# Nightmare-n/GD-MAE

Hardware: AMD Instinct MI355X
Metric: MAE pre-train frames/sec (Waymo-shape, 180k pts, 75% mask) (higher is better)
Workload: dtype bf16

## Files before the change

### gd-mae_amd/csrc/conv_tiles.hip

```cpp
#include "conv_tiles.h"

typedef float f32x16 __attribute__((ext_vector_type(16)));
typedef __bf16 bf16x8 __attribute__((ext_vector_type(8)));
typedef _Float16 f16x8 __attribute__((ext_vector_type(8)));
union CtFrag {
  uint4 q;
  bf16x8 v;
  f16x8 h;
};

#define CT_C 128
#define CT_SITE_PITCH 272
#ifndef CT_CH
#define CT_CH 128
#endif
#ifndef CT_RING
#define CT_RING 8
#endif
#define CT_HALVES (CT_C / CT_CH)
#define CT_KS (CT_CH / 16)
#define CT_NSTEP (9 * CT_KS)
#define CT_CPS (CT_CH / 8)
#define CT_PSITE (CT_CH * 2 + 16)
#define CT_ROW_PITCH (CT_CH == 128 ? 2944 : 1664)
// ... 540 lines not shown
#undef CT_STAGE
  }
  __syncthreads();
  float* red = (float*)(lds + CT_RED_OFF);
  const int elc = tid & 15, elsg = tid >> 4;
#pragma unroll
  for (int t = 0; t < CT_TPW; ++t) {
    if (!have[t]) continue;
    float s[8], q2[8];
#pragma unroll
    for (int j = 0; j < 8; ++j) s[j] = q2[j] = 0.f;
#pragma unroll
    for (int p = 0; p < 64 / CT_ESPP; ++p) {
      const int site = p * CT_ESPP + elsg;
      const uint4 v = *(const uint4*)(lds + t * CT_STAGE_PITCH + site * CT_SITE_PITCH + elc * 16);
      *(uint4*)(A.Yc + ((long long)slot[t] * GD_TILE_SITES + site) * CT_C + elc * 8) = v;
      if (ty0[t] + (site >> 3) < A.H && tx0[t] + (site & 7) < A.W) {
        float f[8];
        ct_unpack8(v, f);
#pragma unroll
        for (int j = 0; j < 8; ++j) {
          s[j] += f[j];
          q2[j] = fmaf(f[j], f[j], q2[j]);
        }
      }
    }
#pragma unroll
    for (int j = 0; j < 8; ++j) {
      s[j] += __shfl_xor(s[j], 16, 64);
      s[j] += __shfl_xor(s[j], 32, 64);
      q2[j] += __shfl_xor(q2[j], 16, 64);
      q2[j] += __shfl_xor(q2[j], 32, 64);
    }
    if (lane < 16) {
#pragma unroll
      for (int j = 0; j < 8; ++j) {
        red[((t * CT_NWAVES + wvg) * 2 + 0) * CT_C + elc * 8 + j] = s[j];
        red[((t * CT_NWAVES + wvg) * 2 + 1) * CT_C + elc * 8 + j] = q2[j];
      }
    }
  }
  __syncthreads();
#pragma unroll
  for (int t = 0; t < CT_TPW; ++t) {
    if (!have[t] || tid >= 256) continue;
    const int stat = tid >> 7, ch = tid & 127;
    float v = 0.f;
#pragma unroll
    for (int w = 0; w < CT_NWAVES; ++w) v += red[((t * CT_NWAVES + w) * 2 + stat) * CT_C + ch];
    A.part[(long long)slot[t] * 256 + tid] = v;
  }
}

__global__ __launch_bounds__(256) void k_ct_stats_reduce(const float* __restrict__ part, int n_act, const int* __restrict__ tile_list,
                                                         const unsigned short* __restrict__ ybg, int B, int H, int W, int TH, int TW,
                                                         float* __restrict__ red) {
  const int tid = threadIdx.x;
  if ((int)blockIdx.x < CT_NRED) {
    const int chunk = (n_act + CT_NRED - 1) / CT_NRED;
    const int r0 = blockIdx.x * chunk, r1 = r0 + chunk < n_act ? r0 + chunk : n_act;
    float a0 = 0.f, a1 = 0.f, a2 = 0.f, a3 = 0.f;
    int r = r0;
    for (; r + 15 < r1; r += 16) {
      float v[16];
#pragma unroll
      for (int u = 0; u < 16; ++u) v[u] = part[(long long)(r + u) * 256 + tid];
#pragma unroll
      for (int u = 0; u < 16; u += 4) {
        a0 += v[u];
        a1 += v[u + 1];
        a2 += v[u + 2];
        a3 += v[u + 3];
      }
    }
    for (; r + 3 < r1; r += 4) {
      a0 += part[(long long)r * 256 + tid];
      a1 += part[(long long)(r + 1) * 256 + tid];
      a2 += part[(long long)(r + 2) * 256 + tid];
      a3 += part[(long long)(r + 3) * 256 + tid];
    }
    for (; r < r1; ++r) a0 += part[(long long)r * 256 + tid];
    red[(long long)blockIdx.x * 256 + tid] = (a0 + a1) + (a2 + a3);
    return;
  }
  __shared__ int cnt[9];
  if (tid < 9) cnt[tid] = 0;
  __syncthreads();
  int c[9];
#pragma unroll
  for (int k = 0; k < 9; ++k) c[k] = 0;
  for (int i0 = tid; i0 < n_act; i0 += 8 * 256) {
   int tl[8];
#pragma unroll
   for (int u = 0; u < 8; ++u) tl[u] = tile_list[i0 + u * 256 < n_act ? i0 + u * 256 : n_act - 1];
#pragma unroll
   for (int u = 0; u < 8; ++u) {
    if (i0 + u * 256 >= n_act) continue;
    const int tile = tl[u];
    const int tx = tile % TW, ty = (tile / TW) % TH;
    const int y0 = ty * 8, y1 = y0 + 8 < H ? y0 + 8 : H, x0 = tx * 8, x1 = x0 + 8 < W ? x0 + 8 : W;
    const int ry[3] = {y0 == 0 ? 1 : 0, 0, y1 == H ? 1 : 0};
    const int rx[3] = {x0 == 0 ? 1 : 0, 0, x1 == W ? 1 : 0};
    const int my = (y1 - y0) - ry[0] - ry[2], mx = (x1 - x0) - rx[0] - rx[2];
#pragma unroll
    for (int cy = 0; cy < 3; ++cy)
#pragma unroll
      for (int cx = 0; cx < 3; ++cx) c[cy * 3 + cx] += (cy == 1 ? my : ry[cy]) * (cx == 1 ? mx : rx[cx]);
   }
  }
#pragma unroll
  for (int k = 0; k < 9; ++k)
    if (c[k]) atomicAdd(&cnt[k], c[k]);
  __syncthreads();
  const int stat = tid >> 7, ch = tid & 127;
  double acc = 0.0;
#pragma unroll
  for (int cy = 0; cy < 3; ++cy)
#pragma unroll
    for (int cx = 0; cx < 3; ++cx) {
      const long long total = (long long)B * (cy == 1 ? H - 2 : 1) * (cx == 1 ? W - 2 : 1);
      const double n = (double)(total - cnt[cy * 3 + cx]);
      const double v = (double)ct_bf2f(ybg[(cy * 3 + cx) * CT_C + ch]);
      acc += n * (stat ? v * v : v);
    }
  const float hi = (float)acc;
  red[(long long)CT_NRED * 256 + tid] = hi;
  red[(long long)(CT_NRED + 1) * 256 + tid] = (float)(acc - (double)hi);
}

int gd_bn_fold_from_partials(hipStream_t st, const float* part, int nblk, int C, double count, const float* gamma,
                             const float* beta, double eps, double momentum, float* running_mean, float* running_var,
                             long long* num_batches, double* stats, float* ab, float* mv);

extern "C" size_t gdmae_conv3x3_tiles_workspace_bytes(int n_act) {
  return gd_align((size_t)(n_act > 0 ? n_act : 1) * 256 * sizeof(float)) + gd_align((size_t)(CT_NRED + 2) * 256 * sizeof(float));
}

static int ct_fwd(const void* const* P, const int* const* maps, const float* const* a, const float* const* b, const int* strides, int k,
                  const void* Wp, const void* ybg, const int* tile_list, int n_act, int B, int H, int W, void* Yc, const float* gamma,
                  const float* beta, double eps, double momentum, float* running_mean, float* running_var, long long* num_batches,
                  double* stats, float* ab, float* mv, const int* tile_class, const int* tile_order, const float* pre, void* workspace,
                  void* stream) {
  GD_REQUIRE(k >= 1 && k <= CT_MAX_SRC, "conv3x3_tiles: 1..3 source stages");
  GD_REQUIRE(H >= 2 && W >= 2, "conv3x3_tiles: map too small");
  hipStream_t st = (hipStream_t)stream;
  CtArgs A;
  A.k = k;
  for (int g = 0; g < CT_MAX_SRC; ++g) {
    if (g < k) {
      const int s = strides[g];
      GD_REQUIRE((s == 1 || s == 2 || s == 4 || s == 8) && H % s == 0 && W % s == 0, "conv3x3_tiles: stride");
      A.src[g].P = (const unsigned short*)P[g];
      A.src[g].map = maps[g];
      A.src[g].a = a[g];
      A.src[g].b = b[g];
      A.src[g].ls = s == 1 ? 0 : (s == 2 ? 1 : (s == 4 ? 2 : 3));
    } else {
      A.src[g].P = nullptr; A.src[g].map = nullptr; A.src[g].a = nullptr; A.src[g].b = nullptr; A.src[g].ls = 0;
    }
  }
  A.Wp = (const uint4*)Wp;
  A.tile_list = tile_list;
  A.n_act = n_act;
  A.H = H; A.W = W; A.TH = (H + 7) / 8; A.TW = (W + 7) / 8;
  A.Yc = (unsigned short*)Yc;
  A.tile_class = CT_SKIP_OK ? tile_class : nullptr;
  A.tile_order = CT_SKIP_OK ? tile_order : nullptr;
  A.pre = CT_SKIP_OK ? pre : nullptr;
  GdArena ar(workspace, gdmae_conv3x3_tiles_workspace_bytes(n_act));
  float* part = ar.take<float>((size_t)(n_act > 0 ? n_act : 1) * 256);
  float* red = ar.take<float>((size_t)(CT_NRED + 2) * 256);
  A.part = part;
  if (n_act > 0) {
    static bool once = false;
    if (!once) {
      GD_CHECK(hipFuncSetAttribute((const void*)k_conv3x3_tiles, hipFuncAttributeMaxDynamicSharedMemorySize, CT_LDS_BYTES));
      once = true;
    }
    hipLaunchKernelGGL(k_conv3x3_tiles, dim3((n_act + CT_TPW - 1) / CT_TPW), dim3(CT_THREADS), CT_LDS_BYTES, st, A);
    GD_LAUNCH_CHECK();
  }
  hipLaunchKernelGGL(k_ct_stats_reduce, dim3(CT_NRED + 1), dim3(256), 0, st, (const float*)part, n_act, tile_list,
                     (const unsigned short*)ybg, B, H, W, A.TH, A.TW, red);
  GD_LAUNCH_CHECK();
  return gd_bn_fold_from_partials(st, red, CT_NRED + 2, CT_C, (double)B * H * W, gamma, beta, eps, momentum, running_mean,
                                  running_var, num_batches, stats, ab, mv);
}

extern "C" int gdmae_conv3x3_tiles_fwd(const void* const* P, const int* const* maps, const float* const* a, const float* const* b,
                                       const int* strides, int k, const void* Wp, const void* ybg, const int* tile_list, int n_act,
                                       int B, int H, int W, void* Yc, const float* gamma, const float* beta, double eps,
                                       double momentum, float* running_mean, float* running_var, long long* num_batches,
                                       double* stats, float* ab, float* mv, void* workspace, void* stream) {
  return ct_fwd(P, maps, a, b, strides, k, Wp, ybg, tile_list, n_act, B, H, W, Yc, gamma, beta, eps, momentum, running_mean, running_var,
                num_batches, stats, ab, mv, nullptr, nullptr, nullptr, workspace, stream);
}

extern "C" int gdmae_conv3x3_tiles_fwd_skip(const void* const* P, const int* const* maps, const float* const* a, const float* const* b,
                                            const int* strides, int k, const void* Wp, const void* ybg, const int* tile_list, int n_act,
                                            int B, int H, int W, void* Yc, const float* gamma, const float* beta, double eps,
                                            double momentum, float* running_mean, float* running_var, long long* num_batches,
                                            double* stats, float* ab, float* mv, const int* tile_class, const int* tile_order,
                                            const float* pre, void* workspace, void* stream) {
  const bool none = !tile_class && !tile_order && !pre;
  GD_REQUIRE(none || (tile_class && tile_order && (pre || k < 2)), "conv3x3_tiles_fwd_skip: tile_class, tile_order and pre, or none of them");
  return ct_fwd(P, maps, a, b, strides, k, Wp, ybg, tile_list, n_act, B, H, W, Yc, gamma, beta, eps, momentum, running_mean, running_var,
                num_batches, stats, ab, mv, tile_class, tile_order, pre, workspace, stream);
}

template <int ES>
__global__ __launch_bounds__(256) void k_tiles_gather_rows(const void* __restrict__ Yc, GdTiles T, const int* __restrict__ cell,
                                                           long long n, int H, int W, int C, uint4* __restrict__ out) {
  const int cv = C * ES / 16;
  const long long total = n * cv;
  for (long long i = blockIdx.x * (long long)blockDim.x + threadIdx.x; i < total; i += (long long)gridDim.x * blockDim.x) {
    const long long r = total < (1ll << 31) ? (long long)((unsigned)i / (unsigned)cv) : i / cv;
    const int v = (int)(i - r * cv);
    const int s = cell[r];
    const int x = s % W, q = s / W, y = q % H, b = q / H;
    out[i] = ((const uint4*)gd_y_row<ES>(Yc, T, b, y, x, H, W, C))[v];
  }
}

extern "C" int gdmae_tiles_gather_rows(const void* Yc, const int* tile_slot, const void* ybg, const int* cell, long long n, int H,
                                       int W, int C, int elem_bytes, void* out, void* stream) {
  GD_REQUIRE(tile_slot != nullptr && (elem_bytes == 2 || elem_bytes == 4) && (C * elem_bytes) % 16 == 0, "tiles_gather_rows");
  if (n <= 0) return 0;
  GdTiles T{tile_slot, ybg, (H + 7) / 8, (W + 7) / 8};
  long long g = (n * (C * elem_bytes / 16) + 255) / 256;
  if (g > 16384) g = 16384;
  if (elem_bytes == 2) hipLaunchKernelGGL(k_tiles_gather_rows<2>, dim3((int)g), dim3(256), 0, (hipStream_t)stream, Yc, T, cell, n, H, W, C, (uint4*)out);
  else hipLaunchKernelGGL(k_tiles_gather_rows<4>, dim3((int)g), dim3(256), 0, (hipStream_t)stream, Yc, T, cell, n, H, W, C, (uint4*)out);
  GD_LAUNCH_CHECK();
  return 0;
}

__global__ __launch_bounds__(256) void k_tiles_gather_rows_affine_relu(const void* __restrict__ Yc, GdTiles T, const int* __restrict__ cell,
                                                                       long long n, int H, int W, int C, const float* __restrict__ a,
                                                                       const float* __restrict__ b, uint4* __restrict__ yrows,
                                                                       float4* __restrict__ out) {
  const int cv = C / 8;
  const long long total = n * cv;
  for (long long i = blockIdx.x * (long long)blockDim.x + threadIdx.x; i < total; i += (long long)gridDim.x * blockDim.x) {
    const long long r = total < (1ll << 31) ? (long long)((unsigned)i / (unsigned)cv) : i / cv;
    const int v = (int)(i - r * cv);
    const int s = cell[r];
    const int x = s % W, q = s / W, y = q % H, bb = q / H;
    const uint4 yq = ((const uint4*)gd_y_row<2>(Yc, T, bb, y, x, H, W, C))[v];
    const float4 a0 = ((const float4*)a)[2 * v], a1 = ((const float4*)a)[2 * v + 1];
    const float4 b0 = ((const float4*)b)[2 * v], b1 = ((const float4*)b)[2 * v + 1];
    const unsigned w4[4] = {yq.x, yq.y, yq.z, yq.w};
    const float av[8] = {a0.x, a0.y, a0.z, a0.w, a1.x, a1.y, a1.z, a1.w};
    const float bv[8] = {b0.x, b0.y, b0.z, b0.w, b1.x, b1.y, b1.z, b1.w};
    float o[8];
#pragma unroll
    for (int j = 0; j < 4; ++j) {
      const float h0 = fmaf(av[2 * j], __uint_as_float(w4[j] << 16), bv[2 * j]);
      const float h1 = fmaf(av[2 * j + 1], __uint_as_float(w4[j] & 0xFFFF0000u), bv[2 * j + 1]);
      o[2 * j] = h0 > 0.f ? h0 : 0.f;
      o[2 * j + 1] = h1 > 0.f ? h1 : 0.f;
// ... 86 lines not shown
```

### gd-mae_amd/gdmae_hip/lib.py

```python
from __future__ import annotations

import ctypes as C
import os

import torch

_HERE = os.path.dirname(os.path.abspath(__file__))
LIB_PATH = os.path.abspath(os.path.join(_HERE, "..", "csrc", "libgdmae_hip.so"))
if os.environ.get("GDMAE_LIB"):
    LIB_PATH = os.path.abspath(os.environ["GDMAE_LIB"])


class GdmaeHipError(RuntimeError):
    pass


_P, _I, _L, _F, _D, _Z = C.c_void_p, C.c_int, C.c_longlong, C.c_float, C.c_double, C.c_size_t

SIGNATURES = {
    "gdmae_abi_version": (_I, []),
    "gdmae_target_arch": (C.c_char_p, []),
    "gdmae_last_error": (C.c_char_p, []),
    "gdmae_voxelize_workspace_bytes": (_Z, [_L, _I, _I, _I, _I]),
    "gdmae_voxelize": (_I, [_P, _L, _I, _P, _P, _P, _I, _P, _P, _P, _P, _P, _P, _P, _P, _P, _P, _P, _P, _P, _P, _Z, _P]),
# ... 4 lines not shown
    "gdmae_vfe_point_layer_fwd": (_I, [_P, _P, _P, _P, _I, _L, _I, _P, _P, _P, _I, _P, _P, _D, _D, _P, _P, _P, _P, _P, _P, _P, _I, _P, _P]),
    "gdmae_vfe_point_layer_bwd": (_I, [_P, _P, _P, _P, _I, _L, _I, _P, _P, _P, _I, _P, _P, _P, _P, _I, _P, _P, _P, _I, _P, _P]),
    "gdmae_vfe_max_layer_workspace_bytes": (_Z, []),
    "gdmae_vfe_max_layer_fwd": (_I, [_P, _L, _P, _P, _P, _I, _P, _P, _D, _D, _P, _P, _P, _P, _P, _P, _P, _P, _P, _P]),
    "gdmae_vfe_max_layer_bwd": (_I, [_P, _L, _P, _P, _I, _P, _P, _P, _P, _P, _P, _P, _P, _P, _P, _P, _I, _P, _P]),
    "gdmae_vfe_max_layer_fwd_f16": (_I, [_P, _L, _P, _P, _P, _I, _P, _P, _D, _D, _P, _P, _P, _P, _P, _P, _P, _P, _P, _P]),
    "gdmae_vfe_max_layer_bwd_f16": (_I, [_P, _L, _P, _P, _I, _P, _P, _P, _P, _P, _P, _P, _P, _P, _P, _P, _I, _P, _P]),
    "gdmae_vfe_max_layer_vis_fwd": (_I, [_P, _L, _P, _P, _P, _L, _I, _P, _P, _D, _D, _P, _P, _P, _P, _P, _P, _P, _P, _P, _P]),
    "gdmae_vfe_max_layer_vis_fwd_f16": (_I, [_P, _L, _P, _P, _P, _L, _I, _P, _P, _D, _D, _P, _P, _P, _P, _P, _P, _P, _P, _P, _P]),
    "gdmae_vfe_max_layer_vis_bwd": (_I, [_P, _L, _P, _P, _P, _I, _I, _P, _P, _P, _P, _P, _P, _P, _P, _P, _P, _P, _I, _P, _P]),
    "gdmae_vfe_max_layer_vis_bwd_f16": (_I, [_P, _L, _P, _P, _P, _I, _I, _P, _P, _P, _P, _P, _P, _P, _P, _P, _P, _P, _I, _P, _P]),
    "gdmae_fill_rows": (_I, [_P, _L, _I, _I, _P, _P]),
    "gdmae_weighted_mean_finish": (_I, [_P, _P, _L, _P, _P]),
    "gdmae_decoder_region_workspace_bytes": (_Z, [_I, _I]),
    "gdmae_decoder_region_algebra": (_I, [_P, _P, _P, _P, _P, _P, _P, _D, _I, _I, _P, _P, _I, _P, _P, _P, _P, _P, _P]),
    "gdmae_segment_max": (_I, [_P, _P, _P, _I, _I, _P, _P, _P]),
    "gdmae_segment_max_bwd": (_I, [_P, _P, _P, _L, _I, _P, _P]),
    "gdmae_random_mask": (_I, [_P, _P, _I, _D, _P, _P, _P]),
    "gdmae_visible_tokens": (_I, [_P, _P, _P, _L, _L, _P, _P, _P, _P, _P, _P]),
    "gdmae_downsample_tokens": (_I, [_P, _P, _L, _I, _I, _I, _P, _P, _P, _P, _P, _P]),
    "gdmae_rulebook": (_I, [_P, _P, _L, _I, _I, _I, _I, _I, _P, _I, _P, _P]),
    "gdmae_window_workspace_bytes": (_Z, [_I, _I, _I, _I, _I]),
    "gdmae_window_partition": (_I, [_P, _I, _I, _I, _I, _I, _I, _I, _P, _P, _P, _P, _P, _P, _P, _P, _P, _P, _P, _P, _Z, _P]),
    "gdmae_gather_rows": (_I, [_P, _P, _L, _I, _P, _P]),
    "gdmae_scatter_rows": (_I, [_P, _P, _L, _I, _P, _P]),
    "gdmae_gather_rows_strided": (_I, [_P, _P, _L, _I, _I, _I, _P, _P]),
    "gdmae_scatter_rows_strided": (_I, [_P, _P, _L, _I, _I, _I, _P, _P]),
    "gdmae_colstats_workspace_bytes": (_Z, [_I]),
    "gdmae_colstats": (_I, [_P, _L, _I, _I, _P, _P, _P]),
    "gdmae_rows_affine_relu_scatter": (_I, [_P, _I, _P, _L, _I, _P, _P, _P, _I, _I, _I, _P]),
    "gdmae_rows_affine_relu_sub": (_I, [_P, _I, _P, _L, _I, _P, _P, _P, _P, _I, _I, _I, _P]),
    "gdmae_rows_affine_relu_add": (_I, [_P, _I, _L, _I, _P, _P, _P, _P, _I, _P]),
    "gdmae_rows_bwd_stats_workspace_bytes": (_Z, [_I]),
    "gdmae_rows_bwd_stats": (_I, [_P, _I, _P, _L, _I, _P, _P, _P, _I, _I, _I, _P, _P, _P]),
    "gdmae_bn_fold": (_I, [_P, _L, _I, _I, _D, _P, _P, _D, _D, _P, _P, _P, _P, _P, _P, _P, _P]),
    "gdmae_bn_bwd_coeffs": (_I, [_P, _I, _P, _P, _P, _I, _D, _P, _P, _P, _I, _P, _P]),
    "gdmae_rows_bwd_stats_rows": (_I, [_L]),
    "gdmae_bn_bwd_coeffs_rows": (_I, [_P, _I, _I, _P, _P, _P, _I, _D, _P, _P, _P, _I, _P, _P]),
    "gdmae_border_sums_workspace_bytes": (_Z, [_I, _I]),
    "gdmae_border_sums": (_I, [_P, _I, _P, _P, _P, _P, _I, _I, _I, _I, _I, _P, _P, _P]),
    "gdmae_border_sums_rows": (_I, [_P, _I, _P, _P, _P, _P, _P, _P, _P, _I, _I, _I, _I, _I, _P, _P, _P]),
    "gdmae_conv3x3_grad_taps": (_I, [_P, _I, _P, _P, _P, _P, _P, _P, _P, _L, _I, _I, _I, _P, _P]),
    "gdmae_decoder_tiles_workspace_bytes": (_Z, [_I, _I, _I]),
    "gdmae_decoder_tiles": (_I, [_P, _P, _I, _I, _I, _I, _P, _P, _P, _P, _P]),
    "gdmae_conv3x3_tiles_packed_bytes": (_Z, [_I]),
    "gdmae_conv3x3_tiles_pack": (_I, [_P, _I, _I, _P, _I, _P, _P, _P, _P]),
    "gdmae_conv3x3_tiles_workspace_bytes": (_Z, [_I]),
    "gdmae_conv3x3_tiles_fwd": (_I, [_P, _P, _P, _P, _P, _I, _P, _P, _P, _I, _I, _I, _I, _P, _P, _P, _D, _D, _P, _P, _P, _P, _P, _P,
                                     _P, _P]),
    "gdmae_decoder_tiles_classes": (_I, [_P, _P, _I, _I, _I, _I, _P, _P, _P, _P, _P, _P, _P]),
    "gdmae_conv3x3_tiles_pack_pre": (_I, [_P, _I, _I, _P, _I, _P, _P, _P, _P, _P]),
    "gdmae_conv3x3_tiles_fwd_skip": (_I, [_P, _P, _P, _P, _P, _I, _P, _P, _P, _I, _I, _I, _I, _P, _P, _P, _D, _D, _P, _P, _P, _P, _P, _P,
                                          _P, _P, _P, _P, _P]),
    "gdmae_tiles_gather_rows": (_I, [_P, _P, _P, _P, _L, _I, _I, _I, _I, _P, _P]),
    "gdmae_tiles_gather_rows_affine_relu": (_I, [_P, _P, _P, _P, _L, _I, _I, _I, _P, _P, _P, _P, _P]),
    "gdmae_tiles_to_dense": (_I, [_P, _P, _P, _I, _I, _I, _I, _I, _P, _P]),
    "gdmae_tiles_to_dense_affine_relu": (_I, [_P, _P, _P, _I, _I, _I, _I, _P, _P, _P, _P]),
    "gdmae_rows_bwd": (_I, [_P, _I, _P, _L, _I, _P, _P, _P, _P, _P, _I, _I, _I, _P, _I, _P]),
    "gdmae_segment_max_affine": (_I, [_P, _I, _P, _P, _I, _I, _P, _P, _P, _P, _P]),
    "gdmae_segmax_bwd_stats": (_I, [_P, _I, _P, _P, _P, _L, _I, _P, _P, _P, _P, _P]),
    "gdmae_segmax_bn_bwd": (_I, [_P, _I, _P, _P, _P, _P, _L, _I, _P, _P, _P, _P, _I, _P]),
    "gdmae_window_attention_fwd": (_I, [_P, _P, _P, _I, _P, _P, _P, _I, _I, _I, _I, _P, _F, _P]),
    "gdmae_window_attention_bwd": (_I, [_P, _P, _P, _P, _P, _I, _P, _P, _P, _P, _I, _I, _I, _I, _P, _F, _P]),
    "gdmae_window_attention_levels_writes_lse": (_I, [_I, _I, _P, _I, _I]),
    "gdmae_window_attention_levels_fwd": (_I, [_P, _P, _P, _I, _P, _P, _P, _I, _P, _P, _I, _I, _P, _F, _P, _P]),
    "gdmae_window_attention_levels_bwd": (_I, [_P, _P, _P, _P, _P, _I, _P, _P, _P, _P, _I, _P, _P, _I, _I, _P, _F, _P, _P, _P]),
    "gdmae_conv3x3_dense_packed_bytes": (_Z, [_I, _I]),
    "gdmae_conv3x3_dense_pack": (_I, [_P, _I, _I, _I, _I, _P, _P]),
    "gdmae_conv3x3_dense": (_I, [_P, _I, _I, _I, _I, _I, _I, _P, _P, _P, _P]),
    "gdmae_conv3x3_dense_add": (_I, [_P, _I, _I, _I, _I, _I, _I, _P, _P, _P, _P, _P]),
    "gdmae_conv3x3_dense_relu": (_I, [_P, _I, _I, _I, _I, _I, _I, _P, _P, _P, _P, _P]),
    "gdmae_conv3x3_dense_stats_workspace_bytes": (_Z, [_I, _I, _I, _I]),
    "gdmae_conv3x3_dense_stat_rows": (_I, []),
    "gdmae_conv3x3_dense_stats": (_I, [_P, _I, _I, _I, _I, _I, _I, _P, _P, _P, _P, _P, _P]),
    "gdmae_bn_fold_partials": (_I, [_P, _I, _I, _D, _P, _P, _D, _D, _P, _P, _P, _P, _P, _P, _P]),
    "gdmae_conv3x3_dense_f32out": (_I, [_P, _I, _I, _I, _I, _I, _I, _P, _P, _P, _I, _P]),
    "gdmae_conv3x3_dense_dw_workspace_bytes": (_Z, [_I, _I, _I, _I, _I]),
    "gdmae_conv3x3_dense_bwd_weight": (_I, [_P, _P, _I, _I, _I, _I, _I, _I, _I, _I, _P, _P, _P]),
    "gdmae_attention_timing": (_I, [_I]),
    "gdmae_attention_timing_read": (_I, [_I, _P, _P]),
    "gdmae_kernel_timing": (_I, [_I]),
    "gdmae_kernel_timing_slots": (_I, []),
    "gdmae_kernel_timing_name": (C.c_char_p, [_I]),
    "gdmae_kernel_timing_read": (_I, [_I, _P, _P, _P, _P]),
    "gdmae_kernel_timing_read_side": (_I, [_I, _P]),
    "gdmae_add_layernorm_workspace_bytes": (_Z, [_I]),
    "gdmae_add_layernorm_fwd": (_I, [_P, _P, _I, _P, _P, _L, _I, _F, _P, _P, _P, _P]),
    "gdmae_add_layernorm_bwd": (_I, [_P, _P, _I, _P, _P, _P, _P, _I, _L, _I, _P, _P, _P, _P, _P]),
    "gdmae_prep_tokens": (_I, [_P, _P, _P, _L, _I, _P, _P, _I, _P]),
    "gdmae_sum_bf16": (_I, [_P, _I, _L, _P, _P]),
    "gdmae_add3": (_I, [_P, _P, _I, _P, _I, _L, _P, _P]),
    "gdmae_add3_to": (_I, [_P, _P, _I, _P, _I, _L, _P, _I, _P]),
    "gdmae_set_attention_impl": (_I, [_I]),
    "gdmae_sum_partials": (_I, [_P, _L, _F, _P, _I, _P]),
    "gdmae_sum_partials_gated": (_I, [_P, _L, _F, _P, _P, _F, _P]),
    "gdmae_gemm_workspace_bytes": (_Z, []),
    "gdmae_gemm_stats": (_I, [_P]),
    "gdmae_gemm_tuning": (_I, [_I]),
    "gdmae_gemm": (_I, [_P, _P, _P, _L, _L, _L, _I, _I, _I, _I, _P, _P, _P]),
    "gdmae_gemm_tn_splitk_workspace_bytes": (_Z, [_L, _I, _I]),
    "gdmae_gemm_tn_splitk": (_I, [_P, _P, _P, _L, _I, _I, _I, _I, _P, _P]),
    "gdmae_conv_block_scratch_bytes": (_Z, [_L, _L, _I, _I, _I]),
    "gdmae_spconv_packed_bytes": (_Z, [_I, _I]),
    "gdmae_spconv_pack_jobs": (_I, [_P, _I, _I, _I, _P, _P]),
    "gdmae_spconv": (_I, [_P, _I, _P, _P, _L, _I, _I, _P, _I, _P]),
    "gdmae_spconv_bias_relu": (_I, [_P, _I, _P, _P, _P, _L, _I, _I, _P, _P]),
# ... 195 lines not shown
```

### include/gdmae_hip.h

```cpp
#ifndef GDMAE_HIP_H
#define GDMAE_HIP_H

#include <stddef.h>
#include <stdint.h>

#ifdef __cplusplus
extern "C" {
#endif

int gdmae_abi_version(void);
const char* gdmae_target_arch(void);
const char* gdmae_last_error(void);

size_t gdmae_voxelize_workspace_bytes(long long n_points, int batch_size, int gx, int gy, int gz);
int gdmae_voxelize(const float* points, long long n_points, int n_cols, const float* lo, const float* vs,
                   const int* grid_xyz, int batch_size, float* points_out, long long* point_coords,
                   long long* inverse, int* inverse32, long long* voxel_coords, int* pillar_cell,
                   int* pillar_pt_off, int* pillar_pts, int* point_rank, int* sample_pillar_off,
                   float* pillar_mean, int* cell2pillar, int* counts, void* workspace, size_t workspace_bytes,
                   void* stream);

int gdmae_decorate_points(const float* points, const long long* point_coords, const int* inverse32,
                          const float* pillar_mean, long long N, int n_cols, const float* lo, const float* vs,
                          float* out, void* stream);
// ... 96 lines not shown
int gdmae_rows_bwd_stats(const void* P, int p_bf16, const int* site, long long n, int C, const float* a, const float* b,
                         const void* dZ, int z_bf16, int z_row_elems, int col0, double* out, void* workspace, void* stream);
int gdmae_rows_bwd(const void* P, int p_bf16, const int* site, long long n, int C, const float* a, const float* b,
                   const float* c0, const float* c1, const void* dZ, int z_bf16, int z_row_elems, int col0, void* dP,
                   int dp_bf16, void* stream);

int gdmae_bn_fold(const void* x, long long R, int C, int is_bf16, double count, const float* gamma, const float* beta,
                  double eps, double momentum, float* running_mean, float* running_var, long long* num_batches,
                  double* stats, float* ab, float* mv, void* workspace, void* stream);
int gdmae_bn_fold_partials(const float* part, int nblk, int C, double count, const float* gamma, const float* beta, double eps,
                           double momentum, float* running_mean, float* running_var, long long* num_batches, double* stats, float* ab,
                           float* mv, void* stream);
int gdmae_bn_bwd_coeffs(const double* st, int n_st, const double* stats, const float* ab, const float* gamma, int C,
                        double count, const double* tot, float* dgamma, float* dbeta, int accumulate, float* c01,
                        void* stream);
int gdmae_rows_bwd_stats_rows(long long n);
int gdmae_bn_bwd_coeffs_rows(const float* part, int nblk, int n_st, const double* stats, const float* ab, const float* gamma, int C,
                             double count, const double* tot, float* dgamma, float* dbeta, int accumulate, float* c01,
                             void* stream);

int gdmae_conv3x3_grad_taps(const void* Y, int y_bf16, const int* tile_slot, const void* ybg, const float* k0,
                            const float* k1, const float* rows, const int* cell2pillar, const int* site, long long n, int H,
                            int W, int C, void* out, void* stream);

size_t gdmae_border_sums_workspace_bytes(int B, int C);
int gdmae_border_sums(const void* Y, int y_bf16, const int* tile_slot, const void* ybg, const float* rows,
                      const int* pillar_cell, int M, int B, int H, int W, int C, double* out, void* workspace, void* stream);
int gdmae_border_sums_rows(const void* Y, int y_bf16, const int* tile_slot, const void* ybg, const float* dout, const void* yrows,
                           const float* a2, const float* b2, const int* pillar_cell, int M, int B, int H, int W, int C, double* out,
                           void* workspace, void* stream);

size_t gdmae_decoder_tiles_workspace_bytes(int B, int H, int W);
int gdmae_decoder_tiles(const int* const* maps, const int* strides, int k, int B, int H, int W, int* tile_slot, int* tile_list,
                        int* n_act, void* workspace, void* stream);
size_t gdmae_conv3x3_tiles_packed_bytes(int k);
int gdmae_conv3x3_tiles_pack(const float* conv_w, int C2, int Cin, const float* const* b, int k, void* Wp, void* bgz, void* ybg,
                             void* stream);
size_t gdmae_conv3x3_tiles_workspace_bytes(int n_act);
int gdmae_conv3x3_tiles_fwd(const void* const* P, const int* const* maps, const float* const* a, const float* const* b,
                            const int* strides, int k, const void* Wp, const void* ybg, const int* tile_list, int n_act, int B,
                            int H, int W, void* Yc, const float* gamma, const float* beta, double eps, double momentum,
                            float* running_mean, float* running_var, long long* num_batches, double* stats, float* ab,
                            float* mv, void* workspace, void* stream);
int gdmae_decoder_tiles_classes(const int* const* maps, const int* strides, int k, int B, int H, int W, int* tile_slot, int* tile_list,
                                int* tile_class, int* tile_order, int* n_act, void* workspace, void* stream);
int gdmae_conv3x3_tiles_pack_pre(const float* conv_w, int C2, int Cin, const float* const* b, int k, void* Wp, void* bgz, void* ybg,
                                 float* pre, void* stream);
int gdmae_conv3x3_tiles_fwd_skip(const void* const* P, const int* const* maps, const float* const* a, const float* const* b,
                                 const int* strides, int k, const void* Wp, const void* ybg, const int* tile_list, int n_act, int B,
                                 int H, int W, void* Yc, const float* gamma, const float* beta, double eps, double momentum,
                                 float* running_mean, float* running_var, long long* num_batches, double* stats, float* ab,
                                 float* mv, const int* tile_class, const int* tile_order, const float* pre, void* workspace,
                                 void* stream);
int gdmae_tiles_gather_rows(const void* Yc, const int* tile_slot, const void* ybg, const int* cell, long long n, int H, int W,
                            int C, int elem_bytes, void* out, void* stream);
int gdmae_tiles_gather_rows_affine_relu(const void* Yc, const int* tile_slot, const void* ybg, const int* cell, long long n, int H, int W,
                                        int C, const float* a, const float* b, void* yrows, float* out, void* stream);
int gdmae_tiles_to_dense(const void* Yc, const int* tile_slot, const void* ybg, int B, int H, int W, int C, int elem_bytes,
                         void* out, void* stream);
int gdmae_tiles_to_dense_affine_relu(const void* Yc, const int* tile_slot, const void* ybg, int B, int H, int W, int C, const float* a,
                                     const float* b, float* out, void* stream);

int gdmae_segment_max_affine(const void* x, int x_bf16, const int* pillar_pt_off, const int* pillar_pts, int M, int C,
                             const float* a, const float* b, float* out, int* arg, void* stream);
int gdmae_segmax_bwd_stats(const void* x, int x_bf16, const float* out, const int* arg, const float* dout, long long M,
                           int C, const float* a ,
                           const float* b, double* sums, void* workspace, void* stream);
int gdmae_segmax_bn_bwd(const void* x, int x_bf16, const float* out, const int* arg, const float* dout,
                        const int* inverse32, long long N, int C, const float* a, const float* c0, const float* c1,
                        void* dx, int dx_bf16, void* stream);

int gdmae_set_attention_impl(int impl);
int gdmae_window_attention_fwd(const void* qk, const void* v, void* out, int io_bf16, const int* csr_tok,
                               const int* win_start, const int* win_len, int n_win, int T, int d, int H,
                               const float* tau, float tau_min, void* stream);
int gdmae_window_attention_bwd(const void* qk, const void* v, const void* dout, void* dqk, void* dv, int io_bf16,
                               float* dtau_part, const int* csr_tok, const int* win_start, const int* win_len,
                               int n_win, int T, int d, int H, const float* tau, float tau_min, void* stream);
int gdmae_window_attention_levels_writes_lse(int io_bf16, int n_levels, const int* max_tokens, int d, int H);
int gdmae_window_attention_levels_fwd(const void* qk, const void* v, void* out, int io_bf16, const int* csr_tok,
                                      const int* win_start, const int* win_len, int n_levels, const int* n_win,
                                      const int* max_tokens, int d, int H, const float* tau, float tau_min, float* lse, void* stream);
int gdmae_window_attention_levels_bwd(const void* qk, const void* v, const void* dout, void* dqk, void* dv, int io_bf16,
                                      float* dtau_part, const int* csr_tok, const int* win_start, const int* win_len,
                                      int n_levels, const int* n_win, const int* max_tokens, int d, int H, const float* tau,
                                      float tau_min, const void* out, const float* lse, void* stream);
int gdmae_attention_timing(int on);
int gdmae_attention_timing_read(int which, double* total_ms, long long* calls);
int gdmae_kernel_timing(int on);
int gdmae_kernel_timing_slots(void);
const char* gdmae_kernel_timing_name(int slot);
int gdmae_kernel_timing_read(int slot, double* total_ms, long long* calls, double* bytes, double* flops);
int gdmae_kernel_timing_read_side(int slot, double* side_bytes);
int gdmae_weighted_mean_finish(const float* term, const float* weights, long long n, float* out, void* stream);
int gdmae_sum_partials(const float* part, long long n, float scale, float* out, int accumulate, void* stream);
int gdmae_sum_partials_gated(const float* part, long long n, float scale, float* out, const float* gate, float gate_min,
                             void* stream);

size_t gdmae_add_layernorm_workspace_bytes(int d);
int gdmae_add_layernorm_fwd(const float* a, const void* b, int b_is_bf16, const float* gamma, const float* beta,
                            long long n, int d, float eps, float* y, float* stats, void* y_bf16 ,
                            void* stream);
int gdmae_add_layernorm_bwd(const float* a, const void* b, int b_is_bf16, const float* gamma, const float* stats,
                            const float* dy, const void* dy2, int dy2_bf16, long long n, int d, float* dx, void* dx_bf16,
                            float* sums, void* workspace, void* stream);
int gdmae_prep_tokens(const float* x, const float* pos_table, const int* tok_pos, long long n, int d, void* x_out,
// ... 349 lines not shown
```

Measured before the change: 1090.

## Add persistent software-pipelined conv3x3 tile kernel overlapping gather with MFMA K-loop

Adds a persistent kernel, launched with one workgroup per CU, that walks tile pairs in a grid-stride loop. The gather and affine-ReLU staging of the next source stage's patch are interleaved into the MFMA K-loop and written to a double-buffered LDS patch. The kernel also prefetches weights through a deep register ring and computes the next tile-pair metadata while the MFMA work runs. The aim is to hide global gather latency and per-workgroup launch and prologue cost behind tensor-core work. In exchange it raises register and LDS pressure, runs at one workgroup per CU, and is enabled by default when skip mode is compiled in, with an environment variable to turn it off.

```diff
diff --git a/gd-mae_amd/csrc/conv_tiles.hip b/gd-mae_amd/csrc/conv_tiles.hip
--- a/gd-mae_amd/csrc/conv_tiles.hip
+++ b/gd-mae_amd/csrc/conv_tiles.hip
@@ -616,6 +616,343 @@
   }
 }
 
+#if CT_SKIP_OK
+#ifndef CT_PSLOTS
+#define CT_PSLOTS 18
+#endif
+#define CT_PDIST (CT_PSLOTS - 1)
+#define CT_PIPE_EPI_OFF (2 * CT_PATCH_BYTES)
+#define CT_PIPE_LDS_BYTES (CT_PIPE_EPI_OFF + CT_EPI_BYTES)
+#define CT_P_AB 13
+#define CT_P_ROWS 14
+#define CT_P_BG 29
+#define CT_P_STAGE 30
+#define CT_P_EVERY 3
+static_assert(CT_NSTEP % CT_PSLOTS == 0, "a k-step must keep its ring slot from phase to phase");
+static_assert(CT_PIPE_LDS_BYTES <= 160 * 1024, "two patch buffers + the epilogue's staging in one CU's LDS");
+static_assert(CT_P_STAGE + CT_P_EVERY * (CT_NPASS - 1) < CT_NSTEP && CT_P_ROWS + CT_NPASS <= CT_P_BG, "the gather's places in the K loop");
+
+struct CtPair {
+  int slot[2], tb[2], ty0[2], tx0[2];
+  int have1, lead;
+};
+struct CtItem {
+  const unsigned short* rows;
+  const int* map;
+  const float *a, *b;
+  int ls, Hs, Ws;
+  int tb[2], ty0[2], tx0[2], have1;
+};
+struct CtPipe {
+  CtFrag wr[CT_PSLOTS];
+  int tokv[CT_NPASS];
+  int aux[CT_NPASS];
+  uint4 q[CT_NPASS];
+  float av[8], bv[8];
+  uint4 bgq;
+  float f[8];
+  uint4 o;
+  int v_ord, v_tile, v_cls, v_r, v_tx, v_ty, v_tb;
+};
+
+__device__ __forceinline__ CtPair ct_pair_make(const CtArgs& A, int p, int s0, int s1, int t0, int t1, int c0, int c1) {
+  CtPair P;
+  P.have1 = 2 * p + 1 < A.n_act;
+  P.slot[0] = s0;
+  P.slot[1] = P.have1 ? s1 : 0;
+  const int tl[2] = {t0, P.have1 ? t1 : 0};
+#pragma unroll
+  for (int t = 0; t < 2; ++t) {
+    P.tx0[t] = (tl[t] % A.TW) * 8;
+    const int r = tl[t] / A.TW;
+    P.ty0[t] = (r % A.TH) * 8;
+    P.tb[t] = r / A.TH;
+  }
+  P.lead = A.tile_class ? (P.have1 && c1 < c0 ? c1 : c0) : 0;
+  return P;
+}
+__device__ __forceinline__ CtPair ct_pair_load(const CtArgs& A, int p) {
+  const int i0 = 2 * p, i1 = i0 + 1 < A.n_act ? i0 + 1 : i0;
+  const int s0 = A.tile_order ? A.tile_order[i0] : i0, s1 = A.tile_order ? A.tile_order[i1] : i1;
+  return ct_pair_make(A, p, s0, s1, A.tile_list[s0], A.tile_list[s1], A.tile_class ? A.tile_class[s0] : 0, A.tile_class ? A.tile_class[s1] : 0);
+}
+__device__ __forceinline__ CtItem ct_item(const CtArgs& A, int g, const CtPair& P) {
+  const CtSrc S = A.src[g];
+  CtItem I;
+  I.rows = S.P ? S.P : (const unsigned short*)S.a;
+  I.map = S.map; I.a = S.a; I.b = S.b; I.ls = S.ls;
+  I.Hs = A.H >> S.ls; I.Ws = A.W >> S.ls;
+#pragma unroll
+  for (int t = 0; t < 2; ++t) { I.tb[t] = P.tb[t]; I.ty0[t] = P.ty0[t]; I.tx0[t] = P.tx0[t]; }
+  I.have1 = P.have1;
+  return I;
+}
+__device__ __forceinline__ void ct_p_lookup(CtPipe& R, const CtItem& I, const CtArgs& A, int gp, int p) {
+  const int t = (gp >> 8) & 1, py = (gp >> 4) & 15, px = gp & 15;
+  const int y = (t ? I.ty0[1] : I.ty0[0]) + py - 1, x = (t ? I.tx0[1] : I.tx0[0]) + px - 1;
+  const bool ok = (((gp >> 9) & ((t ^ 1) | I.have1)) != 0) & ((unsigned)y < (unsigned)A.H) & ((unsigned)x < (unsigned)A.W);
+  const int sm = (1 << I.ls) - 1;
+  R.tokv[p] = I.map[ok ? ((t ? I.tb[1] : I.tb[0]) * I.Hs + (y >> I.ls)) * I.Ws + (x >> I.ls) : 0];
+  R.aux[p] = ok ? ((y & sm) << I.ls) + (x & sm) : -1;
+}
+__device__ __forceinline__ void ct_p_rows(CtPipe& R, const CtItem& I, int lc, int p) {
+  const int tok = R.tokv[p];
+  int c = (tok << (2 * I.ls)) + R.aux[p];
+  c = tok < 0 ? -1 : c;
+  c = R.aux[p] < 0 ? -2 : c;
+  R.aux[p] = c;
+  R.q[p] = *(const uint4*)(I.rows + (long long)(c >= 0 ? c : 0) * CT_C + lc * 8);
+}
+__device__ __forceinline__ void ct_p_ab(CtPipe& R, const CtItem& I, int lc) {
+  const float4 a0 = *(const float4*)(I.a + lc * 8), a1 = *(const float4*)(I.a + lc * 8 + 4);
+  const float4 b0 = *(const float4*)(I.b + lc * 8), b1 = *(const float4*)(I.b + lc * 8 + 4);
+  R.av[0] = a0.x; R.av[1] = a0.y; R.av[2] = a0.z; R.av[3] = a0.w; R.av[4] = a1.x; R.av[5] = a1.y; R.av[6] = a1.z; R.av[7] = a1.w;
+  R.bv[0] = b0.x; R.bv[1] = b0.y; R.bv[2] = b0.z; R.bv[3] = b0.w; R.bv[4] = b1.x; R.bv[5] = b1.y; R.bv[6] = b1.z; R.bv[7] = b1.w;
+}
+__device__ __forceinline__ void ct_p_bg(CtPipe& R) {
+  R.bgq.x = gd_pack_f16_relu(R.bv[0], R.bv[1]); R.bgq.y = gd_pack_f16_relu(R.bv[2], R.bv[3]);
+  R.bgq.z = gd_pack_f16_relu(R.bv[4], R.bv[5]); R.bgq.w = gd_pack_f16_relu(R.bv[6], R.bv[7]);
+}
+__device__ __forceinline__ void ct_p_stage_a(CtPipe& R, int p) {
+  ct_unpack8(R.q[p], R.f);
+#pragma unroll
+  for (int j = 0; j < 8; ++j) R.f[j] = fmaf(R.av[j], R.f[j], R.bv[j]);
+}
+__device__ __forceinline__ void ct_p_stage_b(CtPipe& R) {
+  R.o.x = gd_pack_f16_relu(R.f[0], R.f[1]); R.o.y = gd_pack_f16_relu(R.f[2], R.f[3]);
+  R.o.z = gd_pack_f16_relu(R.f[4], R.f[5]); R.o.w = gd_pack_f16_relu(R.f[6], R.f[7]);
+}
+__device__ __forceinline__ void ct_p_stage_c(const CtPipe& R, unsigned char* dst, int p) {
+  const int c = R.aux[p];
+  uint4 o;
+  o.x = c >= 0 ? R.o.x : (c == -1 ? R.bgq.x : 0u); o.y = c >= 0 ? R.o.y : (c == -1 ? R.bgq.y : 0u);
+  o.z = c >= 0 ? R.o.z : (c == -1 ? R.bgq.z : 0u); o.w = c >= 0 ? R.o.w : (c == -1 ? R.bgq.w : 0u);
+  *(uint4*)dst = o;
+}
+__device__ __forceinline__ void ct_p_stage(CtPipe& R, unsigned char* dst, int p) {
+  ct_p_stage_a(R, p);
+  ct_p_stage_b(R);
+  ct_p_stage_c(R, dst, p);
+}
+
+#define CT_PIPE_PARAMS                                                                                                              \
+  CtPipe &R, CtFrag(&sf)[3][4], f32x16 &acc0, f32x16 &acc1, f32x16 &acc2, f32x16 &acc3, const unsigned char *lb,                    \
+      const uint4 *__restrict__ wp, const uint4 *__restrict__ wpn, const CtItem &I, const CtArgs &A, const int(&geo)[CT_NPASS],     \
+      const int(&loff)[CT_NPASS], unsigned char *dstb, int lc, int lane, int p2, CtPair &N2
+#define CT_PIPE_ARGS R, sf, acc0, acc1, acc2, acc3, lb, wp, wpn, I, A, geo, loff, dstb, lc, lane, p2, N2
+template <bool PF, int st>
+__device__ __forceinline__ void ct_pipe_step(CT_PIPE_PARAMS) {
+  if constexpr (st + CT_PDIST < CT_NSTEP) R.wr[(st + CT_PDIST) % CT_PSLOTS].q = wp[CT_WSTEP(st + CT_PDIST, 0)];
+  else if constexpr (PF) R.wr[(st + CT_PDIST) % CT_PSLOTS].q = wpn[CT_WSTEP(st + CT_PDIST - CT_NSTEP, 0)];
+  if constexpr (st + 2 < CT_NSTEP) {
+    sf[(st + 2) % 3][0].q = *(const uint4*)(lb + CT_OFF(st + 2));
+    sf[(st + 2) % 3][1].q = *(const uint4*)(lb + 4 * CT_ROW_PITCH + CT_OFF(st + 2));
+    sf[(st + 2) % 3][2].q = *(const uint4*)(lb + CT_TILE_PITCH + CT_OFF(st + 2));
+    sf[(st + 2) % 3][3].q = *(const uint4*)(lb + CT_TILE_PITCH + 4 * CT_ROW_PITCH + CT_OFF(st + 2));
+  }
+  if constexpr (PF) {
+    if constexpr (st < CT_NPASS) ct_p_lookup(R, I, A, geo[st], st);
+    if constexpr (st == CT_P_AB) ct_p_ab(R, I, lc);
+    if constexpr (st >= CT_P_ROWS && st < CT_P_ROWS + CT_NPASS) ct_p_rows(R, I, lc, st - CT_P_ROWS);
+    if constexpr (st == CT_P_BG) ct_p_bg(R);
+    if constexpr (st >= CT_P_STAGE && (st - CT_P_STAGE) / 3 < CT_NPASS) {
+      constexpr int p = (st - CT_P_STAGE) / 3, part = (st - CT_P_STAGE) % 3;
+      if constexpr (part == 0) ct_p_stage_a(R, p);
+      if constexpr (part == 1) ct_p_stage_b(R);
+      if constexpr (part == 2) ct_p_stage_c(R, dstb + loff[p], p);
+    }
+    if constexpr (st == 1) {
+      const int i = 2 * p2 + (lane & 1);
+      const int ic = i < A.n_act ? i : A.n_act - 1;
+      const int v = (A.tile_order ? A.tile_order : A.tile_list)[ic];
+      R.v_ord = A.tile_order ? v : ic;
+    }
+    if constexpr (st == 27) {
+      R.v_tile = A.tile_list[R.v_ord];
+      R.v_cls = (A.tile_class ? A.tile_class : A.tile_list)[R.v_ord];
+    }
+    if constexpr (st == CT_P_BG - 1) {
+      R.v_r = R.v_tile / A.TW;
+      R.v_tx = (R.v_tile - R.v_r * A.TW) * 8;
+    }
+    if constexpr (st == CT_P_BG) {
+      R.v_tb = R.v_r / A.TH;
+      R.v_ty = (R.v_r - R.v_tb * A.TH) * 8;
+    }
+    if constexpr (st == CT_NSTEP - 1) {
+      N2.have1 = 2 * p2 + 1 < A.n_act;
+#pragma unroll
+      for (int t = 0; t < 2; ++t) {
+        N2.slot[t] = __builtin_amdgcn_readlane(R.v_ord, t);
+        N2.tx0[t] = __builtin_amdgcn_readlane(R.v_tx, t);
+        N2.ty0[t] = __builtin_amdgcn_readlane(R.v_ty, t);
+        N2.tb[t] = __builtin_amdgcn_readlane(R.v_tb, t);
+      }
+      const int c0 = __builtin_amdgcn_readlane(R.v_cls, 0), c1 = __builtin_amdgcn_readlane(R.v_cls, 1);
+      N2.lead = A.tile_class ? (c1 < c0 ? c1 : c0) : 0;
+    }
+  }
+  acc0 = CT_MFMA(R.wr[st % CT_PSLOTS].h, sf[st % 3][0].h, acc0);
+  acc1 = CT_MFMA(R.wr[st % CT_PSLOTS].h, sf[st % 3][1].h, acc1);
+  acc2 = CT_MFMA(R.wr[st % CT_PSLOTS].h, sf[st % 3][2].h, acc2);
+  acc3 = CT_MFMA(R.wr[st % CT_PSLOTS].h, sf[st % 3][3].h, acc3);
+  __builtin_amdgcn_sched_barrier(0);
+  if constexpr (st + 1 < CT_NSTEP) ct_pipe_step<PF, st + 1>(CT_PIPE_ARGS);
+}
+template <bool PF>
+__device__ __forceinline__ void ct_pipe_kloop(CtPipe& R, f32x16& acc0, f32x16& acc1, f32x16& acc2, f32x16& acc3, const unsigned char* lb,
+                                              const uint4* __restrict__ wp, const uint4* __restrict__ wpn, const CtItem& I, const CtArgs& A,
+                                              const int (&geo)[CT_NPASS], const int (&loff)[CT_NPASS], unsigned char* dstb, int lc, int lane,
+                                              int p2, CtPair& N2) {
+  CtFrag sf[3][4];
+#pragma unroll
+  for (int u = 0; u < 2; ++u) {
+    sf[u][0].q = *(const uint4*)(lb + CT_OFF(u));
+    sf[u][1].q = *(const uint4*)(lb + 4 * CT_ROW_PITCH + CT_OFF(u));
+    sf[u][2].q = *(const uint4*)(lb + CT_TILE_PITCH + CT_OFF(u));
+    sf[u][3].q = *(const uint4*)(lb + CT_TILE_PITCH + 4 * CT_ROW_PITCH + CT_OFF(u));
+  }
+  ct_pipe_step<PF, 0>(CT_PIPE_ARGS);
+}
+
+__global__ __launch_bounds__(256, 1) void k_conv3x3_tiles_pipe(CtArgs A) {
+  extern __shared__ __align__(16) unsigned char lds[];
+  const int tid = threadIdx.x, lane = tid & 63, wv = tid >> 6;
+  const int lc = tid & 15, lsg = tid >> 4;
+  const int npairs = (A.n_act + 1) >> 1, G = gridDim.x;
+  int geo[CT_NPASS], loff[CT_NPASS];
+#pragma unroll
+  for (int p = 0; p < CT_NPASS; ++p) {
+    const int e = p * CT_SPP + lsg;
+    const bool ex = e < 200;
+    const int t = e / 100, r = e - 100 * t, py = r / 10, px = r - py * 10;
+    geo[p] = ex ? (512 | (t << 8) | (py << 4) | px) : 0;
+    loff[p] = ex ? t * CT_TILE_PITCH + py * CT_ROW_PITCH + px * CT_PSITE + lc * 16 : (lc >> 3) * CT_ROW_PITCH + 10 * CT_PSITE + (lc & 7) * 16;
+  }
+  const unsigned char* lbw = lds + ((lane & 31) >> 3) * CT_ROW_PITCH + (lane & 7) * CT_PSITE + (lane >> 5) * 16;
+  const uint4* __restrict__ wbase = A.Wp + wv * 64 + lane;
+
+  int p = blockIdx.x;
+  CtPair cur = ct_pair_load(A, p);
+  bool has_nxt = p + G < npairs;
+  CtPair nxt = ct_pair_load(A, has_nxt ? p + G : p), nxt2 = nxt;
+  CtPipe R;
+  {
+    const uint4* __restrict__ wp = wbase + (size_t)cur.lead * 72 * 256;
+#pragma unroll
+    for (int st = 0; st < CT_PDIST; ++st) R.wr[st].q = wp[CT_WSTEP(st, 0)];
+    const CtItem I = ct_item(A, cur.lead, cur);
+#pragma unroll
+    for (int q = 0; q < CT_NPASS; ++q) ct_p_lookup(R, I, A, geo[q], q);
+    ct_p_ab(R, I, lc);
+#pragma unroll
+    for (int q = 0; q < CT_NPASS; ++q) ct_p_rows(R, I, lc, q);
+    ct_p_bg(R);
+#pragma unroll
+    for (int q = 0; q < CT_NPASS; ++q) ct_p_stage(R, lds + loff[q], q);
+  }
+  __syncthreads();
+  int buf = 0;
+  float* red = (float*)(lds + CT_PIPE_EPI_OFF + CT_RED_OFF);
+  const int elc = tid & 15, elsg = tid >> 4;
+  for (;;) {
+    f32x16 acc0, acc1, acc2, acc3;
+#pragma unroll
+    for (int i = 0; i < 16; ++i) acc0[i] = 0.f;
+    if (cur.lead > 0) {
+      const float* pr = A.pre + (cur.lead - 1) * CT_C + wv * 32 + 4 * (lane >> 5);
+#pragma unroll
+      for (int j = 0; j < 4; ++j) {
+        const float4 v = *(const float4*)(pr + 8 * j);
+        acc0[4 * j] = v.x; acc0[4 * j + 1] = v.y; acc0[4 * j + 2] = v.z; acc0[4 * j + 3] = v.w;
+      }
+    }
+    acc1 = acc2 = acc3 = acc0;
+    for (int g = cur.lead; g < A.k; ++g) {
+      const bool last = g == A.k - 1;
+      const int gn = last ? nxt.lead : g + 1;
+      const CtItem I = ct_item(A, gn, last ? nxt : cur);
+      const uint4* __restrict__ wp = wbase + (size_t)g * 72 * 256;
+      const uint4* __restrict__ wpn = wbase + (size_t)gn * 72 * 256;
+      const unsigned char* lb = lbw + buf * CT_PATCH_BYTES;
+      unsigned char* dstb = lds + (buf ^ 1) * CT_PATCH_BYTES;
+      const int p2 = p + 2 * G < npairs ? p + 2 * G : npairs - 1;
+      if (!last || has_nxt) ct_pipe_kloop<true>(R, acc0, acc1, acc2, acc3, lb, wp, wpn, I, A, geo, loff, dstb, lc, lane, p2, nxt2);
+      else ct_pipe_kloop<false>(R, acc0, acc1, acc2, acc3, lb, wp, wpn, I, A, geo, loff, dstb, lc, lane, p2, nxt2);
+      if (last) {
+        const int n = lane & 31;
+        const int cb = wv * 32 + 4 * (lane >> 5);
+#define CT_STAGE(acc, sb)                                                                                              \
+  _Pragma("unroll") for (int j = 0; j < 4; ++j) {                                                                      \
+    uint2 o;                                                                                                           \
+    o.x = ct_pack2(acc[4 * j], acc[4 * j + 1]);                                                                        \
+    o.y = ct_pack2(acc[4 * j + 2], acc[4 * j + 3]);                                                                    \
+    *(uint2*)(lds + CT_PIPE_EPI_OFF + ((sb) >> 1) * CT_STAGE_PITCH + (((sb) & 1) * 32 + n) * CT_SITE_PITCH + (cb + 8 * j) * 2) = o; \
+  }
+        CT_STAGE(acc0, 0)
+        CT_STAGE(acc1, 1)
+        CT_STAGE(acc2, 2)
+        CT_STAGE(acc3, 3)
+#undef CT_STAGE
+      }
+      __syncthreads();
+      buf ^= 1;
+    }
+#pragma unroll
+    for (int t = 0; t < 2; ++t) {
+      if (t == 1 && !cur.have1) continue;
+      float s[8], q2[8];
+#pragma unroll
+      for (int j = 0; j < 8; ++j) s[j] = q2[j] = 0.f;
+#pragma unroll
+      for (int ps = 0; ps < 64 / CT_ESPP; ++ps) {
+        const int site = ps * CT_ESPP + elsg;
+        const uint4 v = *(const uint4*)(lds + CT_PIPE_EPI_OFF + t * CT_STAGE_PITCH + site * CT_SITE_PITCH + elc * 16);
+        *(uint4*)(A.Yc + ((long long)cur.slot[t] * GD_TILE_SITES + site) * CT_C + elc * 8) = v;
+        if (cur.ty0[t] + (site >> 3) < A.H && cur.tx0[t] + (site & 7) < A.W) {
+          float f[8];
+          ct_unpack8(v, f);
+#pragma unroll
+          for (int j = 0; j < 8; ++j) {
+            s[j] += f[j];
+            q2[j] = fmaf(f[j], f[j], q2[j]);
+          }
+        }
+      }
+#pragma unroll
+      for (int j = 0; j < 8; ++j) {
+        s[j] += __shfl_xor(s[j], 16, 64);
+        s[j] += __shfl_xor(s[j], 32, 64);
+        q2[j] += __shfl_xor(q2[j], 16, 64);
+        q2[j] += __shfl_xor(q2[j], 32, 64);
+      }
+      if (lane < 16) {
+#pragma unroll
+        for (int j = 0; j < 8; ++j) {
+          red[((t * CT_NWAVES + wv) * 2 + 0) * CT_C + elc * 8 + j] = s[j];
+          red[((t * CT_NWAVES + wv) * 2 + 1) * CT_C + elc * 8 + j] = q2[j];
+        }
+      }
+    }
+    __syncthreads();
+#pragma unroll
+    for (int t = 0; t < 2; ++t) {
+      if (t == 1 && !cur.have1) continue;
+      const int stat = tid >> 7, ch = tid & 127;
+      float v = 0.f;
+#pragma unroll
+      for (int w = 0; w < CT_NWAVES; ++w) v += red[((t * CT_NWAVES + w) * 2 + stat) * CT_C + ch];
+      A.part[(long long)cur.slot[t] * 256 + tid] = v;
+    }
+    if (!has_nxt) break;
+    p += G;
+    cur = nxt;
+    nxt = nxt2;
+    has_nxt = p + G < npairs;
+  }
+}
+#endif
+
 __global__ __launch_bounds__(256) void k_ct_stats_reduce(const float* __restrict__ part, int n_act, const int* __restrict__ tile_list,
                                                          const unsigned short* __restrict__ ybg, int B, int H, int W, int TH, int TW,
                                                          float* __restrict__ red) {
@@ -700,12 +1037,27 @@
   return gd_align((size_t)(n_act > 0 ? n_act : 1) * 256 * sizeof(float)) + gd_align((size_t)(CT_NRED + 2) * 256 * sizeof(float));
 }
 
+static int ct_default_schedule() {
+  static const int v = getenv("GDMAE_CT_PIPE") ? atoi(getenv("GDMAE_CT_PIPE")) != 0 : (CT_SKIP_OK ? 1 : 0);
+  return v;
+}
+static int ct_pipe_default_workgroups() {
+  static int n = 0;
+  if (n == 0) {
+    int dev = 0, cus = 0;
+    if (hipGetDevice(&dev) != hipSuccess || hipDeviceGetAttribute(&cus, hipDeviceAttributeMultiprocessorCount, dev) != hipSuccess || cus < 1) cus = 256;
+    n = getenv("GDMAE_CT_PIPE_WGS") && atoi(getenv("GDMAE_CT_PIPE_WGS")) > 0 ? atoi(getenv("GDMAE_CT_PIPE_WGS")) : cus;
+  }
+  return n;
+}
 static int ct_fwd(const void* const* P, const int* const* maps, const float* const* a, const float* const* b, const int* strides, int k,
                   const void* Wp, const void* ybg, const int* tile_list, int n_act, int B, int H, int W, void* Yc, const float* gamma,
                   const float* beta, double eps, double momentum, float* running_mean, float* running_var, long long* num_batches,
                   double* stats, float* ab, float* mv, const int* tile_class, const int* tile_order, const float* pre, void* workspace,
-                  void* stream) {
+                  void* stream, int schedule, int max_workgroups) {
   GD_REQUIRE(k >= 1 && k <= CT_MAX_SRC, "conv3x3_tiles: 1..3 source stages");
+  GD_REQUIRE(schedule == 0 || (schedule == 1 && CT_SKIP_OK), "conv3x3_tiles: schedule 0 (two workgroups per CU, a phase at a time) or 1 (pipelined)");
+  GD_REQUIRE(max_workgroups >= 0, "conv3x3_tiles: max_workgroups");
   GD_REQUIRE(H >= 2 && W >= 2, "conv3x3_tiles: map too small");
   hipStream_t st = (hipStream_t)stream;
   CtArgs A;
@@ -735,15 +1087,25 @@
   float* part = ar.take<float>((size_t)(n_act > 0 ? n_act : 1) * 256);
   float* red = ar.take<float>((size_t)(CT_NRED + 2) * 256);
   A.part = part;
-  if (n_act > 0) {
-    static bool once = false;
-    if (!once) {
-      GD_CHECK(hipFuncSetAttribute((const void*)k_conv3x3_tiles, hipFuncAttributeMaxDynamicSharedMemorySize, CT_LDS_BYTES));
-      once = true;
-    }
+  static bool once = false;
+  if (!once) {
+    GD_CHECK(hipFuncSetAttribute((const void*)k_conv3x3_tiles, hipFuncAttributeMaxDynamicSharedMemorySize, CT_LDS_BYTES));
+#if CT_SKIP_OK
+    GD_CHECK(hipFuncSetAttribute((const void*)k_conv3x3_tiles_pipe, hipFuncAttributeMaxDynamicSharedMemorySize, CT_PIPE_LDS_BYTES));
+#endif
+    once = true;
+  }
+  if (n_act > 0 && schedule == 0) {
     hipLaunchKernelGGL(k_conv3x3_tiles, dim3((n_act + CT_TPW - 1) / CT_TPW), dim3(CT_THREADS), CT_LDS_BYTES, st, A);
     GD_LAUNCH_CHECK();
   }
+#if CT_SKIP_OK
+  if (n_act > 0 && schedule == 1) {
+    const int pairs = (n_act + 1) / 2, cap = max_workgroups > 0 ? max_workgroups : ct_pipe_default_workgroups();
+    hipLaunchKernelGGL(k_conv3x3_tiles_pipe, dim3(pairs < cap ? pairs : cap), dim3(256), CT_PIPE_LDS_BYTES, st, A);
+    GD_LAUNCH_CHECK();
+  }
+#endif
   hipLaunchKernelGGL(k_ct_stats_reduce, dim3(CT_NRED + 1), dim3(256), 0, st, (const float*)part, n_act, tile_list,
                      (const unsigned short*)ybg, B, H, W, A.TH, A.TW, red);
   GD_LAUNCH_CHECK();
@@ -757,7 +1119,7 @@
                                        double momentum, float* running_mean, float* running_var, long long* num_batches,
                                        double* stats, float* ab, float* mv, void* workspace, void* stream) {
   return ct_fwd(P, maps, a, b, strides, k, Wp, ybg, tile_list, n_act, B, H, W, Yc, gamma, beta, eps, momentum, running_mean, running_var,
-                num_batches, stats, ab, mv, nullptr, nullptr, nullptr, workspace, stream);
+                num_batches, stats, ab, mv, nullptr, nullptr, nullptr, workspace, stream, ct_default_schedule(), 0);
 }
 
 extern "C" int gdmae_conv3x3_tiles_fwd_skip(const void* const* P, const int* const* maps, const float* const* a, const float* const* b,
@@ -769,7 +1131,19 @@
   const bool none = !tile_class && !tile_order && !pre;
   GD_REQUIRE(none || (tile_class && tile_order && (pre || k < 2)), "conv3x3_tiles_fwd_skip: tile_class, tile_order and pre, or none of them");
   return ct_fwd(P, maps, a, b, strides, k, Wp, ybg, tile_list, n_act, B, H, W, Yc, gamma, beta, eps, momentum, running_mean, running_var,
-                num_batches, stats, ab, mv, tile_class, tile_order, pre, workspace, stream);
+                num_batches, stats, ab, mv, tile_class, tile_order, pre, workspace, stream, ct_default_schedule(), 0);
+}
+
+extern "C" int gdmae_conv3x3_tiles_fwd_sched(const void* const* P, const int* const* maps, const float* const* a, const float* const* b,
+                                             const int* strides, int k, const void* Wp, const void* ybg, const int* tile_list, int n_act,
+                                             int B, int H, int W, void* Yc, const float* gamma, const float* beta, double eps,
+                                             double momentum, float* running_mean, float* running_var, long long* num_batches,
+                                             double* stats, float* ab, float* mv, const int* tile_class, const int* tile_order,
+                                             const float* pre, void* workspace, void* stream, int schedule, int max_workgroups) {
+  const bool none = !tile_class && !tile_order && !pre;
+  GD_REQUIRE(none || (tile_class && tile_order && (pre || k < 2)), "conv3x3_tiles_fwd_sched: tile_class, tile_order and pre, or none of them");
+  return ct_fwd(P, maps, a, b, strides, k, Wp, ybg, tile_list, n_act, B, H, W, Yc, gamma, beta, eps, momentum, running_mean, running_var,
+                num_batches, stats, ab, mv, tile_class, tile_order, pre, workspace, stream, schedule, max_workgroups);
 }
 
 template <int ES>
diff --git a/gd-mae_amd/gdmae_hip/lib.py b/gd-mae_amd/gdmae_hip/lib.py
--- a/gd-mae_amd/gdmae_hip/lib.py
+++ b/gd-mae_amd/gdmae_hip/lib.py
@@ -80,6 +80,8 @@
     "gdmae_conv3x3_tiles_pack_pre": (_I, [_P, _I, _I, _P, _I, _P, _P, _P, _P, _P]),
     "gdmae_conv3x3_tiles_fwd_skip": (_I, [_P, _P, _P, _P, _P, _I, _P, _P, _P, _I, _I, _I, _I, _P, _P, _P, _D, _D, _P, _P, _P, _P, _P, _P,
                                           _P, _P, _P, _P, _P]),
+    "gdmae_conv3x3_tiles_fwd_sched": (_I, [_P, _P, _P, _P, _P, _I, _P, _P, _P, _I, _I, _I, _I, _P, _P, _P, _D, _D, _P, _P, _P, _P, _P, _P,
+                                           _P, _P, _P, _P, _P, _I, _I]),
     "gdmae_tiles_gather_rows": (_I, [_P, _P, _P, _P, _L, _I, _I, _I, _I, _P, _P]),
     "gdmae_tiles_gather_rows_affine_relu": (_I, [_P, _P, _P, _P, _L, _I, _I, _I, _P, _P, _P, _P, _P]),
     "gdmae_tiles_to_dense": (_I, [_P, _P, _P, _I, _I, _I, _I, _I, _P, _P]),
diff --git a/include/gdmae_hip.h b/include/gdmae_hip.h
--- a/include/gdmae_hip.h
+++ b/include/gdmae_hip.h
@@ -172,6 +172,12 @@
                                  float* running_mean, float* running_var, long long* num_batches, double* stats, float* ab,
                                  float* mv, const int* tile_class, const int* tile_order, const float* pre, void* workspace,
                                  void* stream);
+int gdmae_conv3x3_tiles_fwd_sched(const void* const* P, const int* const* maps, const float* const* a, const float* const* b,
+                                  const int* strides, int k, const void* Wp, const void* ybg, const int* tile_list, int n_act, int B,
+                                  int H, int W, void* Yc, const float* gamma, const float* beta, double eps, double momentum,
+                                  float* running_mean, float* running_var, long long* num_batches, double* stats, float* ab,
+                                  float* mv, const int* tile_class, const int* tile_order, const float* pre, void* workspace,
+                                  void* stream, int schedule, int max_workgroups);
 int gdmae_tiles_gather_rows(const void* Yc, const int* tile_slot, const void* ybg, const int* cell, long long n, int H, int W,
                             int C, int elem_bytes, void* out, void* stream);
 int gdmae_tiles_gather_rows_affine_relu(const void* Yc, const int* tile_slot, const void* ybg, const int* cell, long long n, int H, int W,
```

Result: slower. 1068 (-2.0%).
